# polarlightman/Scoring-rules-for-Gaussian-process-regression-a-new-approach-to-inference

Hardware: AMD Instinct MI355X
Metric: GP fit+predict+CRPS wall-clock (ms) at n=20k full / n=40k FITC; HBM GB/s & MFMA% (higher is better)
Workload: dtype f64; 1 GPU; C3 full GP fit(NLML+LOO-CRPS+LOO-LogS)+predict+score; n=20000, d=8, n_test=5000, kernel=ARD, parallelism=single

## Files before the change

### include/gpscore.h

```cpp
#ifndef GPSCORE_H
#define GPSCORE_H

#include <stdint.h>

#ifdef __cplusplus
extern "C" {
#endif

typedef struct gps_ctx gps_ctx;

enum { GPS_ARD = 0, GPS_RBF = 1 };
enum { GPS_FULL = 0, GPS_LOWER = 1 };

enum {
  GPS_OBJ_NLML = 0,
  GPS_OBJ_LOO_CRPS = 1,
  GPS_OBJ_LOO_LOGS = 2,
  GPS_OBJ_LOGDET = 3,
  GPS_OBJ_QUAD = 4,
  GPS_N_OBJ = 5
};
enum {
  GPS_SC_CRPS = 0, GPS_SC_LOGS = 1, GPS_SC_MSLL = 2, GPS_SC_SMSE = 3,
  GPS_SC_MSE = 4, GPS_SC_COVER = 5, GPS_N_SC = 6
};

#define GPS_ABI_VERSION 900
int gps_version(void);
int gps_build_id(char* out, int cap);
int gps_ctx_create(int device, gps_ctx** out);
int gps_ctx_destroy(gps_ctx* ctx);
const char* gps_last_error(gps_ctx* ctx);
int gps_ctx_set_stream(gps_ctx* ctx, void* hip_stream);
void* gps_ctx_stream(gps_ctx* ctx);
int gps_ctx_synchronize(gps_ctx* ctx);

enum {
  GPS_OPT_OVERLAP = 0,
  GPS_OPT_GEMM_MAP = 3,
  GPS_OPT_TINY_GEMM = 7,
  GPS_OPT_GRAM_REG = 9,
  GPS_OPT_GRAPH = 10,
  GPS_OPT_PRED_PRE = 11,
  GPS_OPT_DAG = 12,
  GPS_OPT_AR_CHUNKS = 15,
  GPS_OPT_DAG_TILES = 13,
  GPS_OPT_STREAM_K = 18,
  GPS_OPT_DAG_WGS = 19,
  GPS_OPT_DAG_GROUP = 17,
  GPS_OPT_SLAB_XCD = 26,
  GPS_OPT_DAG_ORDER = 25,
  GPS_OPT_FITC_DEP = 27,
  GPS_OPT_DAG_TILES_FULL = 28,
  GPS_OPT_DAG_KBATCH = 29,
  GPS_OPT_DAG_TILE_FORM = 30,
  GPS_OPT_GEMM_LIVE = 31,
};
int gps_ctx_set_option(gps_ctx* ctx, int key, int value);

enum { GPS_STAT_GRAPHS = 0, GPS_STAT_GRAPH_CAP = 1, GPS_STAT_GRAPH_OVERFLOW = 2,
       GPS_STAT_DEVICE_BYTES = 3, GPS_STAT_GRAPH_DROPPED = 4, GPS_STAT_GRAPH_EVICTED = 5,
       GPS_N_STATS = 6 };
int gps_ctx_stats(gps_ctx* ctx, int64_t* out, int cap);

int gps_dag_task_list(int T, int flags, uint32_t* out, int cap);
int gps_dag_task_list_ex(int T, int flags, int kb, int kg, uint32_t* out, int cap);
int gps_dag_task_list_tf(int T, int flags, int kb, int kg, int tf, uint32_t* out, int cap);
enum { GPS_DAG_PROTO_ROW = 28 };
int gps_dag_task_protocol(int T, const uint32_t* words, int n, int32_t* out);

typedef struct gps_gemm_desc {
  int32_t lay_a, lay_b, epi;
  int32_t M, N, K;
  int64_t lda, ldb, ldc;
  double alpha, beta;
  int32_t tri, tri_off;
  int32_t lower_out, mirror;
  int32_t kend;
  int32_t tile, ksplit, map_mode;
  int32_t use_ws, sk_alone, dep_mode;
  int32_t reserved;
  int64_t ld_out, c_kslice_stride;
} gps_gemm_desc;
enum { GPS_GEMM_PLAN_TILE = 0, GPS_GEMM_PLAN_KSPLIT = 1, GPS_GEMM_PLAN_MAP = 2,
       GPS_GEMM_PLAN_SK_DP = 3, GPS_GEMM_PLAN_SK_WGS = 4, GPS_GEMM_PLAN_SLAB_XCD = 5,
       GPS_GEMM_PLAN_GRID_X = 6, GPS_GEMM_PLAN_GRID_Y = 7, GPS_N_GEMM_PLAN = 8 };
int gps_gemm_diag_check(const gps_gemm_desc* d, int have_c, int have_kscale, int have_w,
                        const int32_t* kr, int have_out0, int have_out1);
int gps_gemm_diag(gps_ctx* ctx, const gps_gemm_desc* d, const double* A, const double* B,
                  double* C, const double* kscale, const double* w, const int32_t* kr,
                  double* out0, double* out1, int32_t* plan);
int64_t gps_gemm_schedule(const gps_gemm_desc* d, const int32_t* kr, int have_kscale, int slots,
                          int32_t* plan, int32_t* items, int64_t cap);

enum { GPS_POTRF_PLAN_NPAD = 0, GPS_POTRF_PLAN_LEAVES = 1, GPS_POTRF_PLAN_DAGS = 2,
       GPS_POTRF_PLAN_DAG_TMIN = 3, GPS_POTRF_PLAN_DAG_TMAX = 4, GPS_POTRF_PLAN_GEMMS = 5,
       GPS_POTRF_PLAN_REPLAYED = 6, GPS_N_POTRF_PLAN = 8 };
int gps_potrf_diag(gps_ctx* ctx, int64_t n, const double* A, int64_t lda, double* L, double* Linv,
                   double* logdiag, int32_t* info, int32_t* plan);

int gps_grad_terms_diag(gps_ctx* ctx, int which, int obj, int64_t n, int64_t n_pad, int64_t m_pad,
                        double scal, const double* const* in, double* const* out);
int gps_grad_contract_diag(gps_ctx* ctx, int64_t n, int d, const double* X, const double* inv_ell,
                           double sf2, const double* Ainv, const double* Mx, int64_t ld,
                           const double* alpha, const double* v, const double* a, double* out);
int gps_fitc_contract_diag(gps_ctx* ctx, int64_t nr, int64_t nc, int64_t nc_pad, int d,
                           const double* xr, const double* xc, const double* inv_ell, double sf2,
                           int nt, const double* const* R, const int64_t* ldr, const double* coef,
                           const double* const* rs, const double* pc, const double* const* pv,
                           const double* const* qv, double* out, double* zout);

int gps_vec_diag(gps_ctx* ctx, int which, const int64_t* dims, const double* scal,
                 const double* const* in, double* const* out);

int gps_prof_enable(gps_ctx* ctx, int on);
int gps_prof_collect(gps_ctx* ctx, char* json_out, int64_t cap);
int gps_phase_enable(gps_ctx* ctx, int on);
int gps_phase_collect(gps_ctx* ctx, char* json_out, int64_t cap);
int gps_rccl_info(int* version, char* path, int cap);

int gps_gram(gps_ctx* ctx, int kind, const double* X, int64_t n, const double* Xp,
             int64_t m, int d, double log_sf2, const double* log_ell, int n_ell,
             double diag_add, int uplo, double* out);
int gps_potrf(gps_ctx* ctx, int64_t n, double* A, int64_t lda, double* logdet);
int gps_potrs(gps_ctx* ctx, int64_t n, int64_t nrhs, const double* A, int64_t lda,
              const double* B, int64_t ldb, double* X, int64_t ldx);
// ... 186 lines not shown
```

### scoring-rules-for-gaussian-process-regression-a-new-approach-to-inference_amd/csrc/api.hip

```cpp
#include "api_internal.h"

namespace gpsapi {

thread_local std::string g_err;

int fail(gps_ctx* ctx, int code, const std::string& msg) {
  if (ctx) ctx->err = msg;
  g_err = msg;
  return code;
}

hipError_t sync_ctx_streams(gps_ctx* ctx) {
  for (hipStream_t st : {ctx->stream, ctx->side, ctx->aux[0], ctx->aux[1]})
    if (st) {
      const hipError_t e = hipStreamSynchronize(st);
      if (e != hipSuccess) return e;
    }
  return hipSuccess;
}

hipError_t drop_graphs_in(gps_ctx* ctx, const void* p, size_t bytes) {
  if (!ctx || !p || ctx->pgraphs.empty()) return hipSuccess;
  const uintptr_t lo = (uintptr_t)p, hi = lo + bytes;
  bool synced = false;
// ... 106 lines not shown
  if (epi == EPI_ROWSQ || epi == EPI_ROWSQ_DOT) return "gemm_rowsq";
  const int64_t tiles = (int64_t)(p.M / GPS_TILE) * (p.N / GPS_TILE) / (p.lower_out ? 2 : 1);
  const int cls = tiles < 16 ? 0 : (tiles < 256 ? 1 : 2);
  static const char* syrk[3] = {"gemm_syrk_s", "gemm_syrk_m", "gemm_syrk_l"};
  static const char* trmm[3] = {"gemm_trmm_s", "gemm_trmm_m", "gemm_trmm_l"};
  static const char* plain[3] = {"gemm_s", "gemm_m", "gemm_l"};
  if (p.lower_out) return p.ksplit > 1 ? "gemm_syrk_splitk" : syrk[cls];
  return p.tri ? trmm[cls] : plain[cls];
}

double gemm_flops(const GemmParams& p) {
  const double M = p.M, N = p.N, K = p.K;
  if (p.lower_out && p.tri == TRI_K_GE_I) {
    double f = 0.0;
    for (int64_t i = 0; i < p.M; i += GPS_TILE) f += (double)(i + GPS_TILE) * (K - i);
    return 2.0 * GPS_TILE * f;
  }
  if (p.lower_out) return M * (M + 1) * K;
  if ((p.tri == TRI_K_LE_I || p.tri == TRI_K_LE_J) && p.tri_off) {
    const double len = p.tri == TRI_K_LE_I ? M : N, other = p.tri == TRI_K_LE_I ? N : M;
    const double o = p.tri_off, e = std::min<double>(K, o + len);
    return other * (e * e - o * o) + 2.0 * other * K * std::max(0.0, o + len - e);
  }
  if (p.tri) return M * N * K;
  return 2.0 * M * N * K;
}

int gemm(gps_ctx* ctx, int al, int bl, int epi, const GemmParams& p, hipStream_t st,
         GemmLaunchInfo* info) {
  if (!st) st = ctx->stream;
  GemmParams q = p;
  if (q.map_mode == 0) q.map_mode = ctx->fo.gemm_map;
  if (!ctx->fo.gemm_live) q.m_live = q.n_live = 0;
  if (epi == EPI_STORE && (q.ksplit == 1 || q.tile == 64) && !q.ws) {
    DBuf& ws = st == ctx->side      ? ctx->ws_side
               : st == ctx->aux[0] ? ctx->ws_aux[0]
               : st == ctx->aux[1] ? ctx->ws_aux[1]
                                   : ctx->ws_main;
    HIPCHK(ensure(ctx, ws, (size_t)kSplitWsDoubles * 8));
    q.ws = ws.d();
    q.ws_cap = kSplitWsDoubles;
    if (st == ctx->stream && ctx->sk_cnt.p) {
      q.sk_cnt = static_cast<int*>(ctx->sk_cnt.p);
      q.sk_slots = 2 * ctx->ncu;
    }
  }
  std::string tag = gemm_tag(al, bl, epi, p);
  if (ctx->prof > 1) {
    const GemmPlan plan = gemm_plan(epi, q, q.ws ? q.ws_cap : 0);
    char buf[160];
    snprintf(buf, sizeof(buf), " %c%c %dx%dx%d tri%d t%d ks%d ld%lld", al ? 'T' : 'N',
             bl ? 'T' : 'N', p.M, p.N, p.K, (int)p.tri, plan.tile, plan.ksplit, (long long)p.lda);
    tag += buf;
  }
  Prof pr(ctx, tag, gemm_flops(p), 0, st);
  HIPCHK(launch_gemm(al, bl, epi, q, st, info));
  return 0;
}

int gram(gps_ctx* ctx, const char* tag, const double* x, int n, const double* xp, int m, int d,
         const Theta& th, double diag_add, int lower, int pad_identity, double* out, int64_t ldo,
         int M, int N, hipStream_t st) {
  GramParams g;
  memset(&g, 0, sizeof(g));
  g.x = x;
  g.xp = xp;
// ... 528 lines not shown
      ARGCHK(value >= 0 && value <= 2, "GPS_OPT_GRAM_REG must be 0, 1 or 2");
      g_gram_reg = value;
      return 0;
    case GPS_OPT_GRAPH: ctx->graphs = value != 0; return 0;
    case GPS_OPT_PRED_PRE: ctx->pred_pre = value != 0; return 0;
    case GPS_OPT_DAG: ctx->fo.dag = value != 0; return 0;
    case GPS_OPT_DAG_WGS:
      ARGCHK(value >= 0, "GPS_OPT_DAG_WGS must be >= 0");
      ctx->fo.dag_wgs = value;
      return 0;
    case GPS_OPT_FITC_DEP: ctx->fitc_dep = value != 0; return 0;
    case GPS_OPT_DAG_ORDER:
      ARGCHK(value >= 0 && value <= 2, "GPS_OPT_DAG_ORDER must be 0, 1 or 2");
      ctx->dag_order = value;
      return 0;
    case GPS_OPT_DAG_GROUP:
      ARGCHK(value >= 2 && value <= 4, "GPS_OPT_DAG_GROUP must be 2, 3 or 4");
      ctx->fo.dag_group = value;
      return 0;
    case GPS_OPT_DAG_TILES:
      ARGCHK(value >= 2 && value <= 64, "GPS_OPT_DAG_TILES must be in 2..64");
      ctx->fo.dag_tiles = value;
      return 0;
    case GPS_OPT_DAG_TILES_FULL:
      ARGCHK(value == 0 || (value >= 2 && value <= 64), "GPS_OPT_DAG_TILES_FULL must be 0 or in 2..64");
      ctx->fo.dag_tiles_full = value;
      return 0;
    case GPS_OPT_DAG_KBATCH:
      ARGCHK(value >= 0 && (value & 15) <= 8 && (value >> 4 & 15) <= 3 && (value >> 9) == 0,
             "GPS_OPT_DAG_KBATCH must be B | g << 4 [| 256] with B in 0..8 and g in 0..3");
      ctx->fo.dag_kbatch = (value & 15) < 2 ? 0 : value;
      return 0;
    case GPS_OPT_GEMM_LIVE: ctx->fo.gemm_live = value != 0; return 0;
    case GPS_OPT_DAG_TILE_FORM:
      ARGCHK(value >= 0 && (value & 15) <= 8 && (value >> 8) == 0 && ((value & 15) || !value),
             "GPS_OPT_DAG_TILE_FORM must be 0 or minlen | d << 4 with minlen in 1..8 and d in 0..15");
      ctx->fo.dag_tile_form = value;
      return 0;
    default: return fail(ctx, -1, "unknown option");
  }
}

void* gps_ctx_stream(gps_ctx* ctx) { return ctx ? (void*)ctx->stream : nullptr; }

int gps_ctx_synchronize(gps_ctx* ctx) {
  if (int rc = bind(ctx)) return rc;
  HIPCHK(hipStreamSynchronize(ctx->stream));
  return 0;
}

int gps_ctx_stats(gps_ctx* ctx, int64_t* out, int cap) {
  if (int rc = bind(ctx)) return rc;
  ARGCHK(out != nullptr && cap >= 0, "out is NULL or cap < 0");
  size_t bytes = 0;
  for (DBuf* b : ctx_buffers(ctx)) bytes += b->cap;
  int64_t v[GPS_N_STATS];
  v[GPS_STAT_GRAPHS] = (int64_t)ctx->pgraphs.size();
  v[GPS_STAT_GRAPH_CAP] = (int64_t)kMaxGraphs;
  v[GPS_STAT_GRAPH_OVERFLOW] = ctx->graph_overflow;
  v[GPS_STAT_GRAPH_DROPPED] = ctx->graph_dropped;
  v[GPS_STAT_GRAPH_EVICTED] = ctx->graph_evicted;
  v[GPS_STAT_DEVICE_BYTES] = (int64_t)bytes;
  for (int i = 0; i < cap && i < GPS_N_STATS; ++i) out[i] = v[i];
  return GPS_N_STATS;
}

// ... 309 lines not shown
```

### scoring-rules-for-gaussian-process-regression-a-new-approach-to-inference_amd/csrc/api_diag.hip

```cpp
#include "api_internal.h"

static_assert(sizeof(gps_gemm_desc) == 128, "gps_gemm_desc layout");

namespace gpsapi {

struct DiagExtents {
  int64_t a, b, c, kscale, w, kr, out0, out1;
};

static bool diag_check(const gps_gemm_desc& d, bool have_c, bool have_kscale, bool have_w,
                       const int32_t* kr, bool have_out0, bool have_out1, DiagExtents& x,
                       std::string& why) {
#define DIAG_REQ(cond, msg) \
  do {                      \
    if (!(cond)) {          \
      why = msg;            \
      return false;         \
    }                       \
  } while (0)
  DIAG_REQ(d.dep_mode == 0, "dep_mode: the dependent row-norm launch cannot run alone");
  DIAG_REQ((d.lay_a == LAY_N || d.lay_a == LAY_T) && (d.lay_b == LAY_N || d.lay_b == LAY_T),
           "layouts must be 0 or 1");
  DIAG_REQ(d.epi == EPI_STORE || d.epi == EPI_ROWSQ || d.epi == EPI_COLRED || d.epi == EPI_ROWSQ_DOT,
           "unknown epilogue");
// ... 808 lines not shown
}
#undef DIAG_REQ

int64_t gps_gemm_schedule(const gps_gemm_desc* d, const int32_t* kr, int have_kscale, int slots,
                          int32_t* plan, int32_t* items, int64_t cap) {
  if (!d || !plan || cap < 0 || (cap > 0 && !items) || slots < 0 || slots > 4096)
    return fail(nullptr, -1, "gps_gemm_schedule: bad argument");
  DiagExtents x;
  std::string why;
  if (!diag_check(*d, true, have_kscale != 0, true, kr, true, true, x, why))
    return fail(nullptr, -1, "gps_gemm_schedule: " + why);
  static double mark[2];
  GemmParams p = desc_params(*d);
  p.A = p.B = mark; p.C = p.out0 = p.out1 = mark; p.w = mark;
  p.kscale = have_kscale ? mark : nullptr;
  p.kr = d->tri == TRI_KR_J ? kr : nullptr;
  if (own_slabs(*d) || (d->epi == EPI_STORE && (p.ksplit == 1 || p.tile == 64))) {
    p.ws = mark;
    p.ws_cap = kSplitWsDoubles;
    if (!own_slabs(*d) && slots > 0) {
      p.sk_cnt = reinterpret_cast<int*>(mark);
      p.sk_slots = slots;
    }
  }
  GemmLaunchInfo info{};
  const int64_t n = gemm_schedule(d->lay_a, d->lay_b, d->epi, p, info, items, cap);
  if (n < 0) return fail(nullptr, -1, "gps_gemm_schedule: launch_gemm refuses the launch");
  const int v[GPS_N_GEMM_PLAN] = {info.tile, info.ksplit, info.map_mode, info.sk_dp,
                                  info.sk_wgs, info.slab_xcd, info.grid_x, info.grid_y};
  for (int i = 0; i < GPS_N_GEMM_PLAN; ++i) plan[i] = v[i];
  return n;
}

}
```

### scoring-rules-for-gaussian-process-regression-a-new-approach-to-inference_amd/csrc/api_internal.h

```cpp
#pragma once
#include <dlfcn.h>
#include <rccl/rccl.h>
#include <stdio.h>
#include <string.h>

#include <chrono>
#include <climits>
#include <cmath>
#include <condition_variable>
#include <map>
#include <memory>
#include <mutex>
#include <string>
#include <type_traits>
#include <vector>

#include "gps_internal.h"
#include "gpscore.h"

using namespace gps;

namespace gpsapi {


// ... 41 lines not shown
      if (g) {
        (void)hipStreamSynchronize(g);
        (void)hipStreamDestroy(g);
      }
    for (const std::vector<hipEvent_t>* v : {&ready, &done, &staged, &summed})
      for (hipEvent_t e : *v)
        if (e) (void)hipEventDestroy(e);
    for (double* p : stage)
      if (p) (void)hipFree(p);
  }
};

extern std::mutex g_groups_mu;
extern std::map<long long, std::weak_ptr<LocalGroup>> g_groups;

}
using namespace gpsapi;

enum { PRE_NONE = 0, PRE_FITC_Q = 1 };

struct FactorReq {
  int full = 0;
  int half = 0;
  int* sig = nullptr;
  struct Pre {
    int kind = PRE_NONE, n1 = 0;
    int* sig = nullptr;
  } pre;
};
struct FactorOpts {
  int overlap = 1;
  int gemm_map = 0;
  int gemm_live = 1;
  int dag = 1;
  int dag_tiles = 20;
  int dag_tiles_full = 40;
  int dag_kbatch = 8 | 256;
  int dag_tile_form = 2 | 2 << 4;
  int dag_group = 3;
  int dag_wgs = 0;
  int tiny_gemm = 0, stream_k = 0, slab_xcd = 0;
};
static_assert(std::has_unique_object_representations_v<FactorReq> &&
              std::has_unique_object_representations_v<FactorOpts>, "compared as words: no padding");

struct gps_ctx {
  int device = 0;
  hipStream_t stream = nullptr;
  bool own_stream = true;
  hipStream_t side = nullptr;
  hipStream_t aux[2] = {nullptr, nullptr};
  FactorOpts fo;
  int ar_chunks = 4;
  std::vector<hipEvent_t> ar_ev;
  int ncu = 0;
  std::vector<hipEvent_t> sync_ev;
  size_t sync_used = 0;
  bool graphs = true;
  bool pred_pre = true;
  int dag_order = 1;
  bool fitc_dep = true;
  DBuf dsig;
  std::map<int, std::pair<DBuf, int>> dag_lists;
  std::map<uintptr_t, int64_t> zeroed;
  DBuf dag_cnt;
  DBuf sk_cnt;
// ... 197 lines not shown
```

### scoring-rules-for-gaussian-process-regression-a-new-approach-to-inference_amd/csrc/gps_internal.h

```cpp
#pragma once

#include <hip/hip_runtime.h>
#include <stdint.h>

#include <string>
#include <vector>

#include "dag_task.h"

#define GPS_TILE 128
#define GPS_MAX_D 64

namespace gps {

inline int64_t pad_to(int64_t n, int64_t t = GPS_TILE) { return (n + t - 1) / t * t; }

struct GramParams {
  const double* x;
  const double* xp;
  double* out;
  int64_t ldo;
  int n, m;
  int M, N;
  int d;
// ... 15 lines not shown
  TRI_KR_J = 5,
};
enum Epi { EPI_STORE = 0, EPI_ROWSQ = 1, EPI_COLRED = 2, EPI_ROWSQ_DOT = 3 };

struct GemmParams {
  const double* A; int64_t lda;
  const double* B; int64_t ldb;
  double* C; int64_t ldc;
  int64_t c_kslice_stride;
  int M, N, K;
  double alpha, beta;
  const double* kscale;
  const double* w;
  double* out0; double* out1; int64_t ld_out;
  int lower_out;
  int ksplit;
  int tri;
  int tri_off;
  const int* kr;
  int tiles_m, tiles_n;
  int map_mode;
  int tile;
  double* ws;
  int64_t ws_cap;
  int* sk_cnt;
  int sk_slots;
  int sk_dp, sk_wgs;
  int prio;
  int mirror;
  int slab_xcd;
  int kend;
  int m_live, n_live;
  int sk_alone;
  int* dep_sig; int* dep_q; int* dep_err; int dep_grid; int dep_mode;
};
constexpr int kSigStarted = 0;
constexpr int kSigRowCnt = 64;
constexpr int kSigRdy = 128;
constexpr int kSigQueue = 192;
constexpr int kSigInts = kSigQueue + 8 * 64;

struct GemmPlan { int tile, ksplit; };
GemmPlan gemm_plan(int epi, const GemmParams& p, int64_t ws_cap_doubles);
struct GemmLaunchInfo { int tile, ksplit, map_mode, sk_dp, sk_wgs, slab_xcd, grid_x, grid_y; };
extern int g_gram_reg;
extern int g_tiny_gemm;
extern int g_stream_k;
extern int g_slab_xcd;
constexpr int kStreamKTiles = 4096;

#ifdef __HIPCC__
__device__ __forceinline__ double wave_sum(double v) {
#pragma unroll
  for (int o = 32; o > 0; o >>= 1) v += __shfl_xor(v, o);
  return v;
}

template <int NV>
__device__ void block_sum(double (&v)[NV], double* sh) {
  const int lane = threadIdx.x & 63, wave = threadIdx.x >> 6, nw = blockDim.x >> 6;
#pragma unroll
  for (int q = 0; q < NV; ++q) v[q] = wave_sum(v[q]);
  __syncthreads();
  if (lane == 0)
#pragma unroll
    for (int q = 0; q < NV; ++q) sh[q * 16 + wave] = v[q];
// ... 443 lines not shown
```

### scoring-rules-for-gaussian-process-regression-a-new-approach-to-inference_amd/csrc/kernels_gemm.hip

```cpp
#include "gemm_schedule.h"
#include "gps_internal.h"

namespace gps {

typedef double d4 __attribute__((ext_vector_type(4)));
typedef double dv2 __attribute__((ext_vector_type(2)));


__device__ __forceinline__ int dep_band0(int tm, int x) { return (int)((int64_t)tm * x / 8); }
__device__ __forceinline__ int dep_ld(const int* p) {
  return __hip_atomic_load(p, __ATOMIC_RELAXED, __HIP_MEMORY_SCOPE_AGENT);
}
__device__ bool dep_take(const GemmParams& p, double* smem, int& ti, int& tj) {
  const int T = p.tiles_n, tm = p.tiles_m;
  if (p.dep_mode == 2) {
    const int b = (int)blockIdx.x;
    tj = T - 1 - b / tm;
    ti = b - (b / tm) * tm;
    if (tj < 0) return false;
    int x = 7;
    while (x > 0 && dep_band0(tm, x) > ti) --x;
    const int len = dep_band0(tm, x + 1) - dep_band0(tm, x);
    return ti - dep_band0(tm, x) >= min(p.dep_q[x * 64 + tj], len);
  }
// ... 265 lines not shown
      const dv2* src = reinterpret_cast<const dv2*>(p.B + (int64_t)(col0 + j) * p.ldb + k0 + k);
#pragma unroll
      for (int q = 0; q < NQ; ++q) rb[q] = src[q];
    }
  };
  auto store_tile = [&](int buf) {
    double* As = smem + buf * STAGE;
    double* Bs = As + BK * LS;
    if constexpr (ALAY == LAY_T) {
      const int k = tid / TPR, i = (tid % TPR) * 2;
#pragma unroll
      for (int q = 0; q < NQ; ++q) *reinterpret_cast<dv2*>(&As[rowoff(k) + i + 2 * TPR * q]) = ra[q];
    } else {
      const int i = tid / TPI, k = (tid % TPI) * PER;
#pragma unroll
      for (int q = 0; q < NQ; ++q) {
        As[rowoff(k + 2 * q) + i] = ra[q].x;
        As[rowoff(k + 2 * q + 1) + i] = ra[q].y;
      }
    }
    if constexpr (BLAY == LAY_N) {
      const int k = tid / TPR, j = (tid % TPR) * 2;
#pragma unroll
      for (int q = 0; q < NQ; ++q) *reinterpret_cast<dv2*>(&Bs[rowoff(k) + j + 2 * TPR * q]) = rb[q];
    } else {
      const int j = tid / TPI, k = (tid % TPI) * PER;
#pragma unroll
      for (int q = 0; q < NQ; ++q) {
        Bs[rowoff(k + 2 * q) + j] = rb[q].x;
        Bs[rowoff(k + 2 * q + 1) + j] = rb[q].y;
      }
    }
  };

  d4 acc[MI][MI];
#pragma unroll
  for (int mi = 0; mi < MI; ++mi)
#pragma unroll
    for (int ni = 0; ni < MI; ++ni) acc[mi][ni] = (d4){0.0, 0.0, 0.0, 0.0};

  auto compute = [&](int buf) {
    const double* As = smem + buf * STAGE;
    const double* Bs = As + BK * LS;
#pragma unroll
    for (int kk = 0; kk < BK / 4; ++kk) {
      const int krow = rowoff(kk * 4 + (lane >> 4)) + (lane & 15);
      double a[MI], b[MI];
#pragma unroll
      for (int mi = 0; mi < MI; ++mi) a[mi] = As[krow + wr * WT + mi * 16];
#pragma unroll
      for (int ni = 0; ni < MI; ++ni) b[ni] = Bs[krow + wc * WT + ni * 16];
#pragma unroll
      for (int mi = 0; mi < MI; ++mi)
#pragma unroll
        for (int ni = 0; ni < MI; ++ni)
          acc[mi][ni] = __builtin_amdgcn_mfma_f64_16x16x4f64(a[mi], b[ni], acc[mi][ni], 0, 0, 0);
    }
  };

  constexpr bool LIVE = EDGE && (EPI == EPI_STORE || EPI == EPI_COLRED);
  const int mrem = LIVE && p.m_live > 0 ? p.m_live - row0 : TILE;
  const int nrem = LIVE && p.n_live > 0 ? p.n_live - col0 : TILE;
  const bool edge = mrem < TILE || nrem < TILE;
  const int wv = __builtin_amdgcn_readfirstlane(wave);
  const int mi_n = min(MI, max(0, (mrem - (wv >> 1) * WT) >> 4));
  const int ni_n = min(MI, max(0, (nrem - (wv & 1) * WT) >> 4));
  auto compute_edge = [&](int buf) {
    if (mi_n == 0 || ni_n == 0) return;
    const double* As = smem + buf * STAGE;
    const double* Bs = As + BK * LS;
    auto frags = [&](int kk, double (&fa)[MI], double (&fb)[MI]) {
      const int krow = rowoff(kk * 4 + (lane >> 4)) + (lane & 15);
#pragma unroll
      for (int mi = 0; mi < MI; ++mi) fa[mi] = As[krow + wr * WT + mi * 16];
#pragma unroll
      for (int ni = 0; ni < MI; ++ni) fb[ni] = Bs[krow + wc * WT + ni * 16];
    };
#pragma unroll 1
    for (int kk = 0; kk < BK / 4; ++kk) {
      double a[MI], b[MI];
      frags(kk, a, b);
#pragma unroll
      for (int mi = 0; mi < MI; ++mi)
        if (mi < mi_n) {
#pragma unroll
          for (int ni = 0; ni < MI; ++ni)
            if (ni < ni_n)
              acc[mi][ni] = __builtin_amdgcn_mfma_f64_16x16x4f64(a[mi], b[ni], acc[mi][ni], 0, 0, 0);
        }
    }
  };

  const bool rdot = EPI == EPI_ROWSQ_DOT && tj == p.tiles_n - 1 && kb == 0;
  double dacc = 0.0;
  auto row_dot = [&](int buf, int k0) {
    if constexpr (EPI == EPI_ROWSQ_DOT) {
      if (rdot && tid < TILE) {
        const double* As = smem + buf * STAGE;
#pragma unroll
        for (int k = 0; k < BK; ++k) dacc = fma(As[rowoff(k) + tid], p.w[k0 + k], dacc);
      }
    }
  };

  if (nk > 0) {
    load_tile(kb);
    store_tile(0);
    __syncthreads();
    auto mainloop = [&](auto& mma) {
      for (int it = 0; it < nk - 1; ++it) {
        load_tile(kb + (it + 1) * BK);
        if (p.prio) __builtin_amdgcn_s_setprio(1);
        mma(it & 1);
        if (p.prio) __builtin_amdgcn_s_setprio(0);
        row_dot(it & 1, kb + it * BK);
        store_tile((it + 1) & 1);
        __syncthreads();
      }
      mma((nk - 1) & 1);
      row_dot((nk - 1) & 1, kb + (nk - 1) * BK);
    };
    if (!edge) mainloop(compute);
    else mainloop(compute_edge);
  }
  if constexpr (EPI == EPI_ROWSQ_DOT) {
    if (rdot && tid < TILE) p.out1[row0 + tid] = dacc;
  }

  const int lrow = lane >> 4, lcol = lane & 15;
  if constexpr (EPI == EPI_STORE) {
    if (part) {
#pragma unroll
      for (int mi = 0; mi < MI; ++mi)
#pragma unroll
        for (int ni = 0; ni < MI; ++ni)
#pragma unroll
          for (int r = 0; r < 4; ++r) part[((mi * MI + ni) * 4 + r) * 256 + tid] = acc[mi][ni][r];
      return;
    }
    store_acc<TILE>(p, ti, tj, kslice, acc);
  } else if constexpr (EPI == EPI_ROWSQ || EPI == EPI_ROWSQ_DOT) {
    double* red = smem;
    __syncthreads();
#pragma unroll
    for (int mi = 0; mi < MI; ++mi)
#pragma unroll
      for (int r = 0; r < 4; ++r) {
        double s = 0.0;
#pragma unroll
        for (int ni = 0; ni < MI; ++ni) s = fma(acc[mi][ni][r], acc[mi][ni][r], s);
        s += __shfl_xor(s, 1);
        s += __shfl_xor(s, 2);
        s += __shfl_xor(s, 4);
        s += __shfl_xor(s, 8);
        if (lcol == 0) red[wc * TILE + wr * WT + mi * 16 + lrow + 4 * r] = s;
      }
// ... 232 lines not shown
  const int64_t t64 = tiles_for(p, 64);
  const int64_t target = p.lower_out ? 2048 : 1024;
  int ks = 1;
  while (ks < 8 && t64 * ks < target && p.K / (2 * ks) >= 64 &&
         (int64_t)(2 * ks) * p.M * p.N <= ws_cap)
    ks *= 2;
  return {64, ks};
}

hipError_t launch_gemm(int alay, int blay, int epi, const GemmParams& pin, hipStream_t s,
                       GemmLaunchInfo* info, GemmParams* resolved) {
  GemmParams p = pin;
  if (p.M % GPS_TILE || p.N % GPS_TILE || p.K % BK || p.M <= 0 || p.N <= 0)
    return hipErrorInvalidValue;
  if ((p.lda & 1) || (p.ldb & 1) || (p.ldc & 1)) return hipErrorInvalidValue;
  if (p.lower_out && p.M != p.N) return hipErrorInvalidValue;
  if (p.mirror && (!p.lower_out || p.M % 32)) return hipErrorInvalidValue;
  if (p.ksplit < 1) p.ksplit = 1;
  if (p.m_live < 0 || p.m_live > p.M || (p.m_live & 15) || p.n_live < 0 || p.n_live > p.N ||
      (p.n_live & 15))
    return hipErrorInvalidValue;
  if (p.m_live == p.M) p.m_live = 0;
  if (p.n_live == p.N) p.n_live = 0;
  if (p.dep_mode || epi == EPI_ROWSQ || epi == EPI_ROWSQ_DOT) p.m_live = p.n_live = 0;
  if (epi == EPI_ROWSQ_DOT &&
      (!p.w || !p.out1 || p.tri != TRI_K_LE_J || p.tri_off < 0 || p.K != p.tri_off + p.N ||
       p.ksplit != 1))
    return hipErrorInvalidValue;
  const GemmPlan plan = gemm_plan(epi, p, p.ws ? p.ws_cap : 0);
  const int tile = plan.tile;
  if (tile == 16 || tile == 32) {
    if (epi != EPI_STORE || p.kscale) return hipErrorInvalidValue;
    p.m_live = p.n_live = 0;
    const int wpt = plan.ksplit;
    if (wpt != 1 && wpt != 2 && wpt != 4) return hipErrorInvalidValue;
    const int64_t tt = small_tiles(p, tile);
    const dim3 grid((unsigned)((tt * wpt + 3) / 4)), block(256);
    if (info) *info = {tile, wpt, p.map_mode, 0, 0, 0, (int)grid.x, 1};
    if (resolved) {
      *resolved = p;
      return hipSuccess;
    }
    hipError_t err = hipErrorInvalidValue;
#define GPS_SMALL_CASE(AL, BL, RR, W)                                                           \
    if (err == hipErrorInvalidValue && alay == AL && blay == BL && tile == 16 * RR && wpt == W) { \
      hipLaunchKernelGGL((gemm_f64_small_kernel<AL, BL, RR, W>), grid, block, 0, s, p);           \
      err = hipGetLastError();                                                                    \
    }
#define GPS_SMALL_LAYOUTS(RR, W)                                                                \
    GPS_SMALL_CASE(LAY_N, LAY_T, RR, W) GPS_SMALL_CASE(LAY_N, LAY_N, RR, W)                     \
    GPS_SMALL_CASE(LAY_T, LAY_N, RR, W) GPS_SMALL_CASE(LAY_T, LAY_T, RR, W)
    GPS_SMALL_LAYOUTS(1, 1) GPS_SMALL_LAYOUTS(1, 2) GPS_SMALL_LAYOUTS(1, 4)
    GPS_SMALL_LAYOUTS(2, 1) GPS_SMALL_LAYOUTS(2, 2) GPS_SMALL_LAYOUTS(2, 4)
#undef GPS_SMALL_LAYOUTS
#undef GPS_SMALL_CASE
    if (err == hipSuccess && p.mirror) err = launch_sym_mirror(p.C, p.ldc, p.M, s);
    return err;
  }
  if (tile != 64 && tile != 128) return hipErrorInvalidValue;
  if (tile == 64 && epi != EPI_STORE) return hipErrorInvalidValue;
  p.ksplit = plan.ksplit;
  const bool slabbed = p.ksplit > 1 && p.ws != nullptr;
  if (p.ksplit > 1 && !slabbed && (epi != EPI_STORE || p.beta != 0.0)) return hipErrorInvalidValue;
  if (p.ksplit > 1 && !slabbed && p.mirror) return hipErrorInvalidValue;
  GemmParams q = p;
  if (slabbed) {
    if (epi != EPI_STORE) return hipErrorInvalidValue;
    q.C = p.ws;
    q.ldc = p.N;
    q.c_kslice_stride = (int64_t)p.M * p.N;
    q.alpha = 1.0;
    q.beta = 0.0;
  }
  q.tiles_m = q.M / tile;
  q.tiles_n = q.N / tile;
  int tiles = (int)tiles_for(q, tile);
  const bool rowsq = epi == EPI_ROWSQ || epi == EPI_ROWSQ_DOT;
  if (q.dep_mode) {
    if (epi != EPI_ROWSQ || alay != LAY_N || blay != LAY_T || q.tri != TRI_K_LE_J || q.tri_off != 0 ||
        tile != 128 || q.ksplit != 1 || q.tiles_n > 64 || !q.dep_sig || !q.dep_q || !q.dep_err ||
        q.dep_mode > 2 || q.K != q.N)
      return hipErrorInvalidValue;
    q.map_mode = 0;
    q.prio = 0;
    q.slab_xcd = 0;
    q.sk_dp = q.sk_wgs = 0;
    if (resolved) return hipErrorInvalidValue;
    const dim3 grid((unsigned)(q.tiles_m * q.tiles_n)), block(256);
    hipLaunchKernelGGL((gemm_f64_kernel<LAY_N, LAY_T, EPI_ROWSQ, 128>), grid, block, 0, s, q);
    return hipGetLastError();
  }
  const bool pairable = rowsq && q.tri == TRI_K_LE_J && tile == 128 && q.ksplit == 1;
  if (q.map_mode == 6 && !pairable) q.map_mode = 0;
  const bool paired = pairable;
  if (q.map_mode == 0 && q.tri != TRI_NONE && q.tri != TRI_KR_J && !q.lower_out)
    q.map_mode = rowsq ? (paired ? 6 : 5) : 3;
  else if (q.map_mode == 4) q.map_mode = 0;
  if (q.map_mode == 6) tiles = q.tiles_m * ((q.tiles_n + 1) / 2);
  if (q.map_mode == 5 && (q.lower_out || q.tri == TRI_NONE || q.tri == TRI_KR_J)) q.map_mode = 0;
  if (q.map_mode == 5) {
    const bool wi = q.tri == TRI_K_LE_I || q.tri == TRI_K_GE_I;
    const int nb = wi ? q.tiles_n : q.tiles_m, nw = wi ? q.tiles_m : q.tiles_n;
    tiles = 8 * ((nw + 7) / 8) * (((nb + 7) / 8 + 7) / 8) * 64;
  }
  if (q.map_mode == 3) {
    if (q.lower_out || q.tri == TRI_NONE || q.tri == TRI_KR_J) return hipErrorInvalidValue;
    tiles = (q.tri == TRI_K_LE_I || q.tri == TRI_K_GE_I) ? 8 * ((q.tiles_n + 7) / 8) * q.tiles_m
                                                          : 8 * ((q.tiles_m + 7) / 8) * q.tiles_n;
  }
  q.sk_dp = q.sk_wgs = 0;
  if ((g_stream_k == 1 || (g_stream_k == 2 && q.sk_alone)) && epi == EPI_STORE && tile == 128 &&
      q.ksplit == 1 && q.sk_cnt && q.ws &&
      q.sk_slots > 0 && q.tri == TRI_NONE && (q.lower_out || q.map_mode == 0 || q.map_mode == 2)) {
    const int slots = q.sk_slots, rem = tiles % slots;
    if (tiles >= slots && rem > 0 && 4 * rem <= 3 * slots && rem <= kStreamKTiles &&
        (int64_t)(rem + slots) * 128 * 128 <= q.ws_cap && q.K / BK >= 2) {
      q.sk_dp = tiles - rem;
      const int64_t runs = (int64_t)rem * (q.K / BK);
      q.sk_wgs = runs < slots ? (int)runs : slots;
      tiles = q.sk_dp + q.sk_wgs;
    }
  }
  q.prio = (epi == EPI_STORE || epi == EPI_COLRED) && !q.kscale;
  q.slab_xcd = g_slab_xcd && q.ksplit > 1 && q.sk_wgs == 0 &&
               (q.map_mode == 0 || q.map_mode == 2) && (q.lower_out || q.tri == TRI_NONE);
  dim3 grid(tiles, q.ksplit), block(256);
  if (info) *info = {tile, q.ksplit, q.map_mode, q.sk_dp, q.sk_wgs, q.slab_xcd, tiles, q.ksplit};
  if (resolved) {
    *resolved = q;
    return hipSuccess;
  }
  hipError_t err = hipErrorInvalidValue;
#define GPS_GEMM_CASE(AL, BL, EP, T)                                                        \
  if (err == hipErrorInvalidValue && alay == AL && blay == BL && epi == EP && tile == T) { \
    hipLaunchKernelGGL((gemm_f64_kernel<AL, BL, EP, T>), grid, block, 0, s, q);            \
    err = hipGetLastError();                                                                \
  }
  GPS_GEMM_CASE(LAY_N, LAY_T, EPI_STORE, 128)
  GPS_GEMM_CASE(LAY_N, LAY_N, EPI_STORE, 128)
  GPS_GEMM_CASE(LAY_T, LAY_N, EPI_STORE, 128)
  GPS_GEMM_CASE(LAY_T, LAY_T, EPI_STORE, 128)
  GPS_GEMM_CASE(LAY_N, LAY_T, EPI_ROWSQ, 128)
  GPS_GEMM_CASE(LAY_N, LAY_T, EPI_ROWSQ_DOT, 128)
  GPS_GEMM_CASE(LAY_N, LAY_T, EPI_COLRED, 128)
  GPS_GEMM_CASE(LAY_N, LAY_T, EPI_STORE, 64)
  GPS_GEMM_CASE(LAY_N, LAY_N, EPI_STORE, 64)
  GPS_GEMM_CASE(LAY_T, LAY_N, EPI_STORE, 64)
  GPS_GEMM_CASE(LAY_T, LAY_T, EPI_STORE, 64)
#undef GPS_GEMM_CASE
  if (err != hipSuccess) return err;
  if (!slabbed) return p.mirror ? launch_sym_mirror(p.C, p.ldc, p.M, s) : hipSuccess;
  if (p.mirror) {
    const int64_t t32 = p.M / 32;
    hipLaunchKernelGGL(splitk_reduce_sym_kernel, dim3((unsigned)(t32 * (t32 + 1) / 2)), dim3(256), 0,
                       s, p.ws, p.ksplit, p.N, p.alpha, p.beta, p.C, p.ldc);
    return hipGetLastError();
// ... 95 lines not shown
```

### scoring-rules-for-gaussian-process-regression-a-new-approach-to-inference_amd/gpscore/_lib.py

```python
from __future__ import annotations

import ctypes
import os

import numpy as np

_HERE = os.path.dirname(os.path.abspath(__file__))
LIB_PATH = os.environ.get("GPSCORE_LIB", os.path.join(_HERE, "libgpscore.so"))
ABI_VERSION = 900
GPS_N_STATS = 6
GPS_COMM_NONE, GPS_COMM_RCCL, GPS_COMM_LOCAL = 0, 1, 2
COMM_KINDS = {GPS_COMM_NONE: "none", GPS_COMM_RCCL: "rccl", GPS_COMM_LOCAL: "local"}

GPS_ARD, GPS_RBF = 0, 1
GPS_FULL, GPS_LOWER = 0, 1
GPS_OPT_OVERLAP, GPS_OPT_GEMM_MAP, GPS_OPT_TINY_GEMM, GPS_OPT_GRAM_REG = 0, 3, 7, 9
GPS_OPT_GRAPH = 10
GPS_OPT_PRED_PRE = 11
GPS_OPT_DAG = 12
GPS_OPT_DAG_TILES = 13
GPS_OPT_DAG_GROUP = 17
GPS_OPT_STREAM_K = 18
GPS_OPT_DAG_WGS = 19
GPS_OPT_DAG_ORDER = 25
GPS_OPT_SLAB_XCD = 26
GPS_OPT_FITC_DEP = 27
GPS_OPT_DAG_TILES_FULL = 28
GPS_OPT_DAG_KBATCH = 29
GPS_OPT_DAG_TILE_FORM = 30
GPS_OPT_GEMM_LIVE = 31
DAG_TILES_FULL_DEFAULT = 40
DAG_KBATCH_DEFAULT = 8 | 256
DAG_TILE_FORM_DEFAULT = 2 | 2 << 4
GPS_OPT_AR_CHUNKS = 15
OBJ_NAMES = ("nlml", "loo_crps", "loo_logs", "logdet", "quad")
SURFACE_NAMES = ("loo_crps", "insample_crps", "nlml", "loo_logs")
GPS_SURF_LOGS_ADD_NOISE = 1
GPS_BATCH_STALE_NOISE = 1
BATCH_MAX_N, BATCH_MAX_D = 128, 16
BATCH_FITC_MAX_M = 32
BATCH_FITC_TALL_MAX_N = 2048
BATCH_FULL_TALL_MAX_N = 512
BATCH_BLOCK_MAX_FOLDS = 32
BATCH_ES_MAX_FOLD = 128
BATCH_ES_MAX_SIM = 512
SCORE_NAMES = ("test_crps", "test_logs", "test_msll", "test_smse", "test_mse", "test_cover")

_c_int, _c_i64, _c_dbl, _c_vp, _c_cp = (ctypes.c_int, ctypes.c_int64, ctypes.c_double,
                                        ctypes.c_void_p, ctypes.c_char_p)
_P = ctypes.POINTER(ctypes.c_double)

_PI = ctypes.POINTER(ctypes.c_int32)
_PI64 = ctypes.POINTER(ctypes.c_int64)
_PP = ctypes.POINTER(_P)


class GemmDesc(ctypes.Structure):
    _fields_ = [("lay_a", ctypes.c_int32), ("lay_b", ctypes.c_int32), ("epi", ctypes.c_int32),
                ("M", ctypes.c_int32), ("N", ctypes.c_int32), ("K", ctypes.c_int32),
                ("lda", _c_i64), ("ldb", _c_i64), ("ldc", _c_i64),
                ("alpha", _c_dbl), ("beta", _c_dbl),
                ("tri", ctypes.c_int32), ("tri_off", ctypes.c_int32),
                ("lower_out", ctypes.c_int32), ("mirror", ctypes.c_int32),
                ("kend", ctypes.c_int32),
                ("tile", ctypes.c_int32), ("ksplit", ctypes.c_int32), ("map_mode", ctypes.c_int32),
                ("use_ws", ctypes.c_int32), ("sk_alone", ctypes.c_int32),
                ("dep_mode", ctypes.c_int32), ("reserved", ctypes.c_int32),
                ("ld_out", _c_i64), ("c_kslice_stride", _c_i64)]


GEMM_PLAN_NAMES = ("tile", "ksplit", "map_mode", "sk_dp", "sk_wgs", "slab_xcd", "grid_x", "grid_y")
POTRF_PLAN_NAMES = ("n_pad", "leaves", "dags", "dag_tmin", "dag_tmax", "gemms", "replayed",
                    "reserved")

SIGNATURES = {
    "gps_version": (_c_int, []),
    "gps_build_id": (_c_int, [_c_cp, _c_int]),
    "gps_ctx_create": (_c_int, [_c_int, ctypes.POINTER(_c_vp)]),
    "gps_ctx_destroy": (_c_int, [_c_vp]),
    "gps_last_error": (_c_cp, [_c_vp]),
    "gps_ctx_set_stream": (_c_int, [_c_vp, _c_vp]),
    "gps_ctx_stream": (_c_vp, [_c_vp]),
    "gps_ctx_synchronize": (_c_int, [_c_vp]),
    "gps_ctx_set_option": (_c_int, [_c_vp, _c_int, _c_int]),
    "gps_ctx_stats": (_c_int, [_c_vp, _c_vp, _c_int]),
    "gps_dag_task_list": (_c_int, [_c_int, _c_int, _c_vp, _c_int]),
    "gps_dag_task_list_ex": (_c_int, [_c_int, _c_int, _c_int, _c_int, _c_vp, _c_int]),
    "gps_dag_task_list_tf": (_c_int, [_c_int, _c_int, _c_int, _c_int, _c_int, _c_vp, _c_int]),
    "gps_dag_task_protocol": (_c_int, [_c_int, _c_vp, _c_int, _PI]),
    "gps_gemm_diag_check": (_c_int, [ctypes.POINTER(GemmDesc), _c_int, _c_int, _c_int, _PI, _c_int,
                                     _c_int]),
    "gps_gemm_schedule": (_c_i64, [ctypes.POINTER(GemmDesc), _PI, _c_int, _c_int, _PI, _PI, _c_i64]),
    "gps_gemm_diag": (_c_int, [_c_vp, ctypes.POINTER(GemmDesc), _P, _P, _P, _P, _P, _PI, _P, _P,
                               _PI]),
    "gps_potrf_diag": (_c_int, [_c_vp, _c_i64, _P, _c_i64, _P, _P, _P, _PI, _PI]),
    "gps_grad_terms_diag": (_c_int, [_c_vp, _c_int, _c_int, _c_i64, _c_i64, _c_i64, _c_dbl, _PP,
                                     _PP]),
    "gps_grad_contract_diag": (_c_int, [_c_vp, _c_i64, _c_int, _P, _P, _c_dbl, _P, _P, _c_i64, _P,
                                        _P, _P, _P]),
    "gps_fitc_contract_diag": (_c_int, [_c_vp, _c_i64, _c_i64, _c_i64, _c_int, _P, _P, _P, _c_dbl,
                                        _c_int, _PP, _PI64, _P, _PP, _P, _PP, _PP, _P, _P]),
    "gps_vec_diag": (_c_int, [_c_vp, _c_int, _PI64, _P, _PP, _PP]),
    "gps_prof_enable": (_c_int, [_c_vp, _c_int]),
    "gps_prof_collect": (_c_int, [_c_vp, _c_cp, _c_i64]),
    "gps_phase_enable": (_c_int, [_c_vp, _c_int]),
    "gps_phase_collect": (_c_int, [_c_vp, _c_cp, _c_i64]),
    "gps_rccl_info": (_c_int, [ctypes.POINTER(_c_int), _c_cp, _c_int]),
    "gps_gram": (_c_int, [_c_vp, _c_int, _P, _c_i64, _P, _c_i64, _c_int, _c_dbl, _P, _c_int,
                          _c_dbl, _c_int, _P]),
    "gps_potrf": (_c_int, [_c_vp, _c_i64, _P, _c_i64, _P]),
    "gps_potrs": (_c_int, [_c_vp, _c_i64, _c_i64, _P, _c_i64, _P, _c_i64, _P, _c_i64]),
    "gps_diag_inv": (_c_int, [_c_vp, _c_i64, _P, _c_i64, _P]),
    "gps_gemm": (_c_int, [_c_vp, _c_int, _c_int, _c_i64, _c_i64, _c_i64, _c_dbl, _P, _c_i64, _P,
                          _c_i64, _c_dbl, _P, _c_i64]),
    "gps_scores": (_c_int, [_c_vp, _P, _P, _P, _c_i64, _c_dbl, _c_dbl, _P]),
    "gps_full_set_data": (_c_int, [_c_vp, _P, _P, _c_i64, _c_int]),
    "gps_full_set_test": (_c_int, [_c_vp, _P, _P, _c_i64]),
    "gps_full_fit": (_c_int, [_c_vp, _c_int, _P, _c_int, _P, _P, _P]),
    "gps_full_grad": (_c_int, [_c_vp, _c_int, _P, _c_int, _c_int, _P, _P]),
    "gps_full_predict": (_c_int, [_c_vp, _P, _P, _P]),
    "gps_fitc_set_data": (_c_int, [_c_vp, _P, _P, _c_i64, _c_int, _c_dbl, _c_dbl, _c_i64]),
    "gps_fitc_set_test": (_c_int, [_c_vp, _P, _P, _c_i64, _c_i64]),
    "gps_fitc_set_inducing": (_c_int, [_c_vp, _P, _c_i64]),
    "gps_fitc_fit": (_c_int, [_c_vp, _P, _c_int, _P, _P, _P]),
    "gps_fitc_grad": (_c_int, [_c_vp, _P, _c_int, _c_int, _P, _P, _P]),
# ... 373 lines not shown
```

Baseline: 8.670 fit+predict+score units/s (C3 full GP, whole job).

## Add software-pipelined GEMM mainloop interleaving LDS traffic with MFMA via scheduling barriers

```diff
diff --git a/include/gpscore.h b/include/gpscore.h
--- a/include/gpscore.h
+++ b/include/gpscore.h
@@ -55,6 +55,7 @@
   GPS_OPT_DAG_KBATCH = 29,
   GPS_OPT_DAG_TILE_FORM = 30,
   GPS_OPT_GEMM_LIVE = 31,
+  GPS_OPT_GEMM_PIPE = 32,
 };
 int gps_ctx_set_option(gps_ctx* ctx, int key, int value);
 
@@ -92,6 +93,7 @@
                   double* out0, double* out1, int32_t* plan);
 int64_t gps_gemm_schedule(const gps_gemm_desc* d, const int32_t* kr, int have_kscale, int slots,
                           int32_t* plan, int32_t* items, int64_t cap);
+int gps_gemm_pipe_resolved(const gps_gemm_desc* d, const int32_t* kr, int have_kscale, int pipe);
 
 enum { GPS_POTRF_PLAN_NPAD = 0, GPS_POTRF_PLAN_LEAVES = 1, GPS_POTRF_PLAN_DAGS = 2,
        GPS_POTRF_PLAN_DAG_TMIN = 3, GPS_POTRF_PLAN_DAG_TMAX = 4, GPS_POTRF_PLAN_GEMMS = 5,
diff --git a/scoring-rules-for-gaussian-process-regression-a-new-approach-to-inference_amd/csrc/api.hip b/scoring-rules-for-gaussian-process-regression-a-new-approach-to-inference_amd/csrc/api.hip
--- a/scoring-rules-for-gaussian-process-regression-a-new-approach-to-inference_amd/csrc/api.hip
+++ b/scoring-rules-for-gaussian-process-regression-a-new-approach-to-inference_amd/csrc/api.hip
@@ -162,6 +162,7 @@
   GemmParams q = p;
   if (q.map_mode == 0) q.map_mode = ctx->fo.gemm_map;
   if (!ctx->fo.gemm_live) q.m_live = q.n_live = 0;
+  q.pipe = ctx->fo.gemm_pipe;
   if (epi == EPI_STORE && (q.ksplit == 1 || q.tile == 64) && !q.ws) {
     DBuf& ws = st == ctx->side      ? ctx->ws_side
                : st == ctx->aux[0] ? ctx->ws_aux[0]
@@ -756,6 +757,7 @@
       ctx->fo.dag_kbatch = (value & 15) < 2 ? 0 : value;
       return 0;
     case GPS_OPT_GEMM_LIVE: ctx->fo.gemm_live = value != 0; return 0;
+    case GPS_OPT_GEMM_PIPE: ctx->fo.gemm_pipe = value != 0; return 0;
     case GPS_OPT_DAG_TILE_FORM:
       ARGCHK(value >= 0 && (value & 15) <= 8 && (value >> 8) == 0 && ((value & 15) || !value),
              "GPS_OPT_DAG_TILE_FORM must be 0 or minlen | d << 4 with minlen in 1..8 and d in 0..15");
diff --git a/scoring-rules-for-gaussian-process-regression-a-new-approach-to-inference_amd/csrc/api_diag.hip b/scoring-rules-for-gaussian-process-regression-a-new-approach-to-inference_amd/csrc/api_diag.hip
--- a/scoring-rules-for-gaussian-process-regression-a-new-approach-to-inference_amd/csrc/api_diag.hip
+++ b/scoring-rules-for-gaussian-process-regression-a-new-approach-to-inference_amd/csrc/api_diag.hip
@@ -864,4 +864,27 @@
   return n;
 }
 
-}
+int gps_gemm_pipe_resolved(const gps_gemm_desc* d, const int32_t* kr, int have_kscale, int pipe) {
+  if (!d) return fail(nullptr, -1, "gps_gemm_pipe_resolved: bad argument");
+  DiagExtents x;
+  std::string why;
+  if (!diag_check(*d, true, have_kscale != 0, true, kr, true, true, x, why))
+    return fail(nullptr, -1, "gps_gemm_pipe_resolved: " + why);
+  static double mark[2];
+  GemmParams p = desc_params(*d);
+  p.A = p.B = mark; p.C = p.out0 = p.out1 = mark; p.w = mark;
+  p.kscale = have_kscale ? mark : nullptr;
+  p.kr = d->tri == TRI_KR_J ? kr : nullptr;
+  if (own_slabs(*d) || (d->epi == EPI_STORE && (p.ksplit == 1 || p.tile == 64))) {
+    p.ws = mark;
+    p.ws_cap = kSplitWsDoubles;
+  }
+  p.pipe = pipe;
+  GemmLaunchInfo info{};
+  GemmParams q;
+  if (launch_gemm(d->lay_a, d->lay_b, d->epi, p, nullptr, &info, &q) != hipSuccess)
+    return fail(nullptr, -1, "gps_gemm_pipe_resolved: launch_gemm refuses the launch");
+  return q.pipe;
+}
+
+}
diff --git a/scoring-rules-for-gaussian-process-regression-a-new-approach-to-inference_amd/csrc/api_internal.h b/scoring-rules-for-gaussian-process-regression-a-new-approach-to-inference_amd/csrc/api_internal.h
--- a/scoring-rules-for-gaussian-process-regression-a-new-approach-to-inference_amd/csrc/api_internal.h
+++ b/scoring-rules-for-gaussian-process-regression-a-new-approach-to-inference_amd/csrc/api_internal.h
@@ -97,6 +97,7 @@
   int overlap = 1;
   int gemm_map = 0;
   int gemm_live = 1;
+  int gemm_pipe = 1;
   int dag = 1;
   int dag_tiles = 20;
   int dag_tiles_full = 40;
diff --git a/scoring-rules-for-gaussian-process-regression-a-new-approach-to-inference_amd/csrc/gps_internal.h b/scoring-rules-for-gaussian-process-regression-a-new-approach-to-inference_amd/csrc/gps_internal.h
--- a/scoring-rules-for-gaussian-process-regression-a-new-approach-to-inference_amd/csrc/gps_internal.h
+++ b/scoring-rules-for-gaussian-process-regression-a-new-approach-to-inference_amd/csrc/gps_internal.h
@@ -71,6 +71,7 @@
   int kend;
   int m_live, n_live;
   int sk_alone;
+  int pipe;
   int* dep_sig; int* dep_q; int* dep_err; int dep_grid; int dep_mode;
 };
 constexpr int kSigStarted = 0;
diff --git a/scoring-rules-for-gaussian-process-regression-a-new-approach-to-inference_amd/csrc/kernels_gemm.hip b/scoring-rules-for-gaussian-process-regression-a-new-approach-to-inference_amd/csrc/kernels_gemm.hip
--- a/scoring-rules-for-gaussian-process-regression-a-new-approach-to-inference_amd/csrc/kernels_gemm.hip
+++ b/scoring-rules-for-gaussian-process-regression-a-new-approach-to-inference_amd/csrc/kernels_gemm.hip
@@ -321,6 +321,60 @@
       }
     }
   };
+  auto load_plain = [&](int k0) {
+    if constexpr (ALAY == LAY_T) {
+      const int k = tid / TPR, i = (tid % TPR) * 2;
+      const dv2* src = reinterpret_cast<const dv2*>(p.A + (int64_t)(k0 + k) * p.lda + row0 + i);
+#pragma unroll
+      for (int q = 0; q < NQ; ++q) ra[q] = src[q * TPR];
+    } else {
+      const int i = tid / TPI, k = (tid % TPI) * PER;
+      const dv2* src = reinterpret_cast<const dv2*>(p.A + (int64_t)(row0 + i) * p.lda + k0 + k);
+#pragma unroll
+      for (int q = 0; q < NQ; ++q) ra[q] = src[q];
+    }
+    if constexpr (BLAY == LAY_N) {
+      const int k = tid / TPR, j = (tid % TPR) * 2;
+      const dv2* src = reinterpret_cast<const dv2*>(p.B + (int64_t)(k0 + k) * p.ldb + col0 + j);
+#pragma unroll
+      for (int q = 0; q < NQ; ++q) rb[q] = src[q * TPR];
+    } else {
+      const int j = tid / TPI, k = (tid % TPI) * PER;
+      const dv2* src = reinterpret_cast<const dv2*>(p.B + (int64_t)(col0 + j) * p.ldb + k0 + k);
+#pragma unroll
+      for (int q = 0; q < NQ; ++q) rb[q] = src[q];
+    }
+  };
+  auto store_a = [&](int buf) {
+    double* As = smem + buf * STAGE;
+    if constexpr (ALAY == LAY_T) {
+      const int k = tid / TPR, i = (tid % TPR) * 2;
+#pragma unroll
+      for (int q = 0; q < NQ; ++q) *reinterpret_cast<dv2*>(&As[rowoff(k) + i + 2 * TPR * q]) = ra[q];
+    } else {
+      const int i = tid / TPI, k = (tid % TPI) * PER;
+#pragma unroll
+      for (int q = 0; q < NQ; ++q) {
+        As[rowoff(k + 2 * q) + i] = ra[q].x;
+        As[rowoff(k + 2 * q + 1) + i] = ra[q].y;
+      }
+    }
+  };
+  auto store_b = [&](int buf) {
+    double* Bs = smem + buf * STAGE + BK * LS;
+    if constexpr (BLAY == LAY_N) {
+      const int k = tid / TPR, j = (tid % TPR) * 2;
+#pragma unroll
+      for (int q = 0; q < NQ; ++q) *reinterpret_cast<dv2*>(&Bs[rowoff(k) + j + 2 * TPR * q]) = rb[q];
+    } else {
+      const int j = tid / TPI, k = (tid % TPI) * PER;
+#pragma unroll
+      for (int q = 0; q < NQ; ++q) {
+        Bs[rowoff(k + 2 * q) + j] = rb[q].x;
+        Bs[rowoff(k + 2 * q + 1) + j] = rb[q].y;
+      }
+    }
+  };
 
   d4 acc[MI][MI];
 #pragma unroll
@@ -348,6 +402,7 @@
   };
 
   constexpr bool LIVE = EDGE && (EPI == EPI_STORE || EPI == EPI_COLRED);
+  constexpr bool PIPE = LIVE && TILE == 128;
   const int mrem = LIVE && p.m_live > 0 ? p.m_live - row0 : TILE;
   const int nrem = LIVE && p.n_live > 0 ? p.n_live - col0 : TILE;
   const bool edge = mrem < TILE || nrem < TILE;
@@ -409,8 +464,79 @@
       mma((nk - 1) & 1);
       row_dot((nk - 1) & 1, kb + (nk - 1) * BK);
     };
-    if (!edge) mainloop(compute);
-    else mainloop(compute_edge);
+    auto mainloop_pipe = [&]() {
+      constexpr int DSR = 0x100, DSW = 0x200, MFMA = 0x8;
+      auto frags = [&](const double* As, const double* Bs, int kk, double (&fa)[MI], double (&fb)[MI]) {
+        const int krow = rowoff(kk * 4 + (lane >> 4)) + (lane & 15);
+#pragma unroll
+        for (int mi = 0; mi < MI; ++mi) fa[mi] = As[krow + wr * WT + mi * 16];
+#pragma unroll
+        for (int ni = 0; ni < MI; ++ni) fb[ni] = Bs[krow + wc * WT + ni * 16];
+      };
+      auto mmas = [&](const double (&fa)[MI], const double (&fb)[MI]) {
+#pragma unroll
+        for (int mi = 0; mi < MI; ++mi)
+#pragma unroll
+          for (int ni = 0; ni < MI; ++ni)
+            acc[mi][ni] = __builtin_amdgcn_mfma_f64_16x16x4f64(fa[mi], fb[ni], acc[mi][ni], 0, 0, 0);
+      };
+      auto pin = [&](auto reads, auto stores) {
+        constexpr int R = decltype(reads)::value ? 4 : 0, W = decltype(stores)::value ? 8 : 0;
+#pragma unroll
+        for (int g = 0; g < R; ++g) {
+          __builtin_amdgcn_sched_group_barrier(DSR, 2, 0);
+          __builtin_amdgcn_sched_group_barrier(MFMA, 1, 0);
+        }
+#pragma unroll
+        for (int g = 0; g < W; ++g) {
+          __builtin_amdgcn_sched_group_barrier(DSW, 1, 0);
+          __builtin_amdgcn_sched_group_barrier(MFMA, 1, 0);
+        }
+        __builtin_amdgcn_sched_group_barrier(MFMA, 16 - R - W, 0);
+      };
+      constexpr std::true_type yes{};
+      constexpr std::false_type no{};
+      for (int it = 0; it < nk - 1; ++it) {
+        const double* As = smem + (it & 1) * STAGE;
+        const double* Bs = As + BK * LS;
+        const int nb = (it + 1) & 1;
+        double a0[MI], b0[MI], a1[MI], b1[MI];
+        frags(As, Bs, 0, a0, b0);
+        __builtin_amdgcn_sched_barrier(0);
+        load_plain(kb + (it + 1) * BK);
+        __builtin_amdgcn_sched_barrier(0);
+        __builtin_amdgcn_s_setprio(1);
+        frags(As, Bs, 1, a1, b1);
+        mmas(a0, b0);
+        pin(yes, no);
+        __builtin_amdgcn_sched_barrier(0);
+        frags(As, Bs, 2, a0, b0);
+        mmas(a1, b1);
+        pin(yes, no);
+        __builtin_amdgcn_sched_barrier(0);
+        frags(As, Bs, 3, a1, b1);
+        store_a(nb);
+        mmas(a0, b0);
+        pin(yes, yes);
+        __builtin_amdgcn_sched_barrier(0);
+        store_b(nb);
+        mmas(a1, b1);
+        pin(no, yes);
+        __builtin_amdgcn_sched_barrier(0);
+        __builtin_amdgcn_s_setprio(0);
+        __syncthreads();
+      }
+      compute((nk - 1) & 1);
+    };
+    bool piped = false;
+    if constexpr (PIPE) piped = p.pipe && !edge && !p.kscale && p.prio;
+    if (piped) {
+      if constexpr (PIPE) mainloop_pipe();
+    } else if (!edge) {
+      mainloop(compute);
+    } else {
+      mainloop(compute_edge);
+    }
   }
   if constexpr (EPI == EPI_ROWSQ_DOT) {
     if (rdot && tid < TILE) p.out1[row0 + tid] = dacc;
@@ -709,6 +835,7 @@
   if (tile == 16 || tile == 32) {
     if (epi != EPI_STORE || p.kscale) return hipErrorInvalidValue;
     p.m_live = p.n_live = 0;
+    p.pipe = 0;
     const int wpt = plan.ksplit;
     if (wpt != 1 && wpt != 2 && wpt != 4) return hipErrorInvalidValue;
     const int64_t tt = small_tiles(p, tile);
@@ -760,6 +887,7 @@
       return hipErrorInvalidValue;
     q.map_mode = 0;
     q.prio = 0;
+    q.pipe = 0;
     q.slab_xcd = 0;
     q.sk_dp = q.sk_wgs = 0;
     if (resolved) return hipErrorInvalidValue;
@@ -799,6 +927,7 @@
     }
   }
   q.prio = (epi == EPI_STORE || epi == EPI_COLRED) && !q.kscale;
+  q.pipe = q.pipe != 0 && tile == 128 && q.prio;
   q.slab_xcd = g_slab_xcd && q.ksplit > 1 && q.sk_wgs == 0 &&
                (q.map_mode == 0 || q.map_mode == 2) && (q.lower_out || q.tri == TRI_NONE);
   dim3 grid(tiles, q.ksplit), block(256);
diff --git a/scoring-rules-for-gaussian-process-regression-a-new-approach-to-inference_amd/gpscore/_lib.py b/scoring-rules-for-gaussian-process-regression-a-new-approach-to-inference_amd/gpscore/_lib.py
--- a/scoring-rules-for-gaussian-process-regression-a-new-approach-to-inference_amd/gpscore/_lib.py
+++ b/scoring-rules-for-gaussian-process-regression-a-new-approach-to-inference_amd/gpscore/_lib.py
@@ -29,6 +29,7 @@
 GPS_OPT_DAG_KBATCH = 29
 GPS_OPT_DAG_TILE_FORM = 30
 GPS_OPT_GEMM_LIVE = 31
+GPS_OPT_GEMM_PIPE = 32
 DAG_TILES_FULL_DEFAULT = 40
 DAG_KBATCH_DEFAULT = 8 | 256
 DAG_TILE_FORM_DEFAULT = 2 | 2 << 4
@@ -91,6 +92,7 @@
     "gps_gemm_diag_check": (_c_int, [ctypes.POINTER(GemmDesc), _c_int, _c_int, _c_int, _PI, _c_int,
                                      _c_int]),
     "gps_gemm_schedule": (_c_i64, [ctypes.POINTER(GemmDesc), _PI, _c_int, _c_int, _PI, _PI, _c_i64]),
+    "gps_gemm_pipe_resolved": (_c_int, [ctypes.POINTER(GemmDesc), _PI, _c_int, _c_int]),
     "gps_gemm_diag": (_c_int, [_c_vp, ctypes.POINTER(GemmDesc), _P, _P, _P, _P, _P, _PI, _P, _P,
                                _PI]),
     "gps_potrf_diag": (_c_int, [_c_vp, _c_i64, _P, _c_i64, _P, _P, _P, _PI, _PI]),
```

Measured after the change: 8.847 fit+predict+score units/s (C3 full GP, whole job), median of 6. 2.0% higher.
